# MayDomine/Burst-Attention

Hardware: NVIDIA H100
Metric: attention fwd+bwd TFLOPS/s (bs=1, H=32, d=128, bf16; seq in config, default 262144 on N > 1 GPUs, 65536 on one), aggregate over GPUs (higher is better)
Workload: dtype bf16

## Files before the change

burst-attention_b200/csrc/fwd_sm90.cuh:

```cuda
#pragma once
#include <math.h>
#include <stdlib.h>

#include "host_common.h"
#include "sm90_ptx.cuh"

namespace ba {

constexpr int kBlockM = 128;
constexpr int kBlockN = 128;
constexpr int kKStages = 2;
constexpr int kVStages = 2;
constexpr int kBoxBytes = 128 * 64 * 2;
constexpr int kFwdThreads = 384;

struct FwdParams {
  float* o_acc;
  int64_t oacc_sb, oacc_ss, oacc_sh;
  float* lse;
  int64_t lse_sb, lse_sh;
  void* o_out;
  int64_t oout_sb, oout_ss, oout_sh;
  int B, Sq, Sk, H;
  int G;
  float scale_log2;
  const float* bias;
  int64_t bias_sb, bias_sh;
  int causal;
  int causal_off;
  int load_state;
  int store_lowp;
  int lo;
};

struct __align__(8) FwdBarriers {
  uint64_t q_full;
  uint64_t k_full[kKStages], k_empty[kKStages];
  uint64_t b_full[kKStages];
  uint64_t v_full[kVStages], v_empty[kVStages];
};

template <int kD>
struct FwdLayout {
  static_assert(kD == 64 || kD == 128, "head dim 64 or 128");
  static constexpr uint32_t kTileB = 128 * kD * 2;
  static constexpr int kBoxes = kD / 64;
  static constexpr uint32_t kOffQ = 0;
  static constexpr uint32_t kOffK = kTileB;
  static constexpr uint32_t kOffV = kOffK + kKStages * kTileB;
  static constexpr uint32_t kOffBias = kOffV + kVStages * kTileB;
  static constexpr uint32_t kOffBars = kOffBias + kKStages * kBlockN * 4;
  static constexpr int kSmemBytes = kOffBars + 256 ;
  static_assert(kSmemBytes <= 232448, "forward kernel exceeds 227 KiB of shared memory");
};

__device__ __forceinline__ int fwd_trip_count(int r0, const FwdParams& p) {
  if (r0 >= p.Sq) return 0;
  int r_last = min(r0 + 63, p.Sq - 1);
  int max_limit = p.causal ? min(r_last + p.causal_off, p.Sk - 1) : p.Sk - 1;
  return max_limit < 0 ? 0 : max_limit / kBlockN + 1;
}

__device__ __forceinline__ int fwd_first_tile(int r0, const FwdParams& p) { return max(0, r0 + p.lo) / kBlockN; }

template <bool kBF16, int kD, bool kBias, bool kBand>
__global__ void __launch_bounds__(kFwdThreads, 1)
fwd_chunk_kernel(const __grid_constant__ CUtensorMap tmQ, const __grid_constant__ CUtensorMap tmK,
                 const __grid_constant__ CUtensorMap tmV, const FwdParams p) {
  extern __shared__ __align__(1024) uint8_t smem_raw[];
  uint8_t* smem = smem_raw;
  if ((smem_u32(smem) & 1023u) != 0) __trap();
  using L = FwdLayout<kD>;
  constexpr uint32_t kTileBytes = L::kTileB;
  constexpr int kBoxes = L::kBoxes, kOReg = kD / 2;
  uint8_t* sQ = smem + L::kOffQ;
  uint8_t* sK = smem + L::kOffK;
  uint8_t* sV = smem + L::kOffV;
  float* sBias = reinterpret_cast<float*>(smem + L::kOffBias);
  FwdBarriers* bars = reinterpret_cast<FwdBarriers*>(smem + L::kOffBars);

  const int warp = __shfl_sync(0xffffffffu, threadIdx.x >> 5, 0);
  const int lane = threadIdx.x & 31;
  const int h = blockIdx.y, b = blockIdx.z;
  const int row0 = (p.causal ? (int)(gridDim.x - 1 - blockIdx.x) : (int)blockIdx.x) * kBlockM;
  int n_tiles = max(fwd_trip_count(row0, p), fwd_trip_count(row0 + 64, p));
  int t0 = 0;
  if constexpr (kBand) {
    t0 = min(fwd_first_tile(row0, p), n_tiles);
    n_tiles -= t0;
  }

  if (threadIdx.x == 0) {
    tma_prefetch_desc(&tmQ);
    tma_prefetch_desc(&tmK);
    tma_prefetch_desc(&tmV);
    mbar_init(&bars->q_full, 1);
    for (int i = 0; i < kKStages; ++i) {
      mbar_init(&bars->k_full[i], 1);
      mbar_init(&bars->k_empty[i], 8);
      mbar_init(&bars->b_full[i], 1);
    }
    for (int i = 0; i < kVStages; ++i) {
      mbar_init(&bars->v_full[i], 1);
      mbar_init(&bars->v_empty[i], 8);
    }
    fence_mbar_init();
  }
  __syncthreads();

  if (warp < 4) {
    reg_alloc_dec<40>();
    if (warp != 0) return;
    const int hk = h / p.G;
    if (lane == 0) {
      mbar_arrive_expect_tx(&bars->q_full, kTileBytes);
      for (int half = 0; half < kBoxes; ++half)
        tma_load_4d(sQ + half * kBoxBytes, &tmQ, &bars->q_full, half * 64, h, row0, b);
    }
    for (int i = 0; i < n_tiles; ++i) {
      const int ks = i % kKStages, kph = (i / kKStages) & 1;
      mbar_wait(&bars->k_empty[ks], kph ^ 1);
      if (lane == 0) {
        mbar_arrive_expect_tx(&bars->k_full[ks], kTileBytes);
        for (int half = 0; half < kBoxes; ++half)
          tma_load_4d(sK + ks * kTileBytes + half * kBoxBytes, &tmK, &bars->k_full[ks], half * 64, hk,
                      (t0 + i) * kBlockN, b);
      }
      if constexpr (kBias) {
#pragma unroll
        for (int j = 0; j < 4; ++j) {
          const int key = (t0 + i) * kBlockN + lane + 32 * j;
          float x = 0.f;
          if (key < p.Sk) x = __ldg(p.bias + (int64_t)b * p.bias_sb + (int64_t)h * p.bias_sh + key) * kLog2e;
          sBias[ks * kBlockN + lane + 32 * j] = x;
        }
        __syncwarp();
        if (lane == 0) mbar_arrive(&bars->b_full[ks]);
      }
      if (lane == 0) {
        const int vs = i % kVStages, vph = (i / kVStages) & 1;
        mbar_wait(&bars->v_empty[vs], vph ^ 1);
        mbar_arrive_expect_tx(&bars->v_full[vs], kTileBytes);
        for (int half = 0; half < kBoxes; ++half)
          tma_load_4d(sV + vs * kTileBytes + half * kBoxBytes, &tmV, &bars->v_full[vs], half * 64, hk,
                      (t0 + i) * kBlockN, b);
      }
      __syncwarp();
    }
    return;
  }

  reg_alloc_inc<232>();
  const int wg = (threadIdx.x >> 7) - 1;
  const int w = warp & 3, g = lane >> 2, t = lane & 3;
  const int r_lo = row0 + wg * 64 + 16 * w + g;
  const int rows[2] = {r_lo, r_lo + 8};
  const int n_mine = fwd_trip_count(row0 + wg * 64, p);
  const float scale_log2 = p.scale_log2;
  int limit[2];
#pragma unroll
  for (int r = 0; r < 2; ++r) limit[r] = p.causal ? min(rows[r] + p.causal_off, p.Sk - 1) : p.Sk - 1;
  const int limit_min = min(limit[0], limit[1]);
  int my0 = 0, lo_limit[2] = {0, 0};
  if constexpr (kBand) {
    my0 = fwd_first_tile(row0 + wg * 64, p);
    lo_limit[0] = rows[0] + p.lo;
    lo_limit[1] = rows[1] + p.lo;
  }
  const int lo_limit_max = max(lo_limit[0], lo_limit[1]);

  float o[kOReg];
  float m[2] = {-INFINITY, -INFINITY}, l[2] = {0.f, 0.f};
#pragma unroll
  for (int i = 0; i < kOReg; ++i) o[i] = 0.f;
  if (p.load_state) {
#pragma unroll
    for (int r = 0; r < 2; ++r) {
      if (rows[r] >= p.Sq) continue;
      const float lse_prev = p.lse[(int64_t)b * p.lse_sb + (int64_t)h * p.lse_sh + rows[r]];
      if (lse_prev != -INFINITY) {
        m[r] = lse_prev * kLog2e;
        l[r] = t == 0 ? 1.f : 0.f;
      }
      const float* src = p.o_acc + (int64_t)b * p.oacc_sb + (int64_t)rows[r] * p.oacc_ss + (int64_t)h * p.oacc_sh;
#pragma unroll
      for (int c = 0; c < kD / 8; ++c) {
        const float2 f = __ldg(reinterpret_cast<const float2*>(src + 8 * c + 2 * t));
        o[4 * c + 2 * r] = f.x;
        o[4 * c + 2 * r + 1] = f.y;
      }
    }
  }

  const uint32_t q_base = smem_u32(sQ) + wg * 64 * 128;
  mbar_wait(&bars->q_full, 0);
  for (int i = 0; i < n_tiles; ++i) {
    const int ks = i % kKStages, kph = (i / kKStages) & 1;
    const int vs = i % kVStages, vph = (i / kVStages) & 1;
    const bool work = kBand ? (t0 + i >= my0 && t0 + i < n_mine) : i < n_mine;
    mbar_wait(&bars->k_full[ks], kph);
    float sc[64];
    if (work) {
      const uint32_t k_base = smem_u32(sK + ks * kTileBytes);
      wgmma_fence();
#pragma unroll
      for (int kk = 0; kk < kD / 16; ++kk) {
        const uint32_t off = (kk >> 2) * kBoxBytes + (kk & 3) * 32;
        wgmma_ss_n128<kBF16, 0, 0>(sc, make_desc(q_base + off, 16, 1024), make_desc(k_base + off, 16, 1024),
                                   kk > 0 ? 1u : 0u);
      }
      wgmma_commit();
      wgmma_wait<0>();
      fence_regs<64>(sc);
      const int key0 = (t0 + i) * kBlockN;
      if constexpr (kBias) {
        mbar_wait(&bars->b_full[ks], kph);
        const float* bias = sBias + ks * kBlockN;
#pragma unroll
        for (int c = 0; c < 16; ++c) {
          const float2 bb = *reinterpret_cast<const float2*>(bias + 8 * c + 2 * t);
#pragma unroll
          for (int r = 0; r < 2; ++r) {
            sc[4 * c + 2 * r] = fmaf(sc[4 * c + 2 * r], scale_log2, bb.x);
            sc[4 * c + 2 * r + 1] = fmaf(sc[4 * c + 2 * r + 1], scale_log2, bb.y);
          }
        }
      } else {
#pragma unroll
        for (int j = 0; j < 64; ++j) sc[j] *= scale_log2;
      }
      if (key0 + kBlockN - 1 > limit_min) {
#pragma unroll
        for (int c = 0; c < 16; ++c)
#pragma unroll
          for (int e = 0; e < 4; ++e)
            if (key0 + 8 * c + 2 * t + (e & 1) > limit[e >> 1]) sc[4 * c + e] = -INFINITY;
      }
      if constexpr (kBand) {
        if (key0 < lo_limit_max) {
#pragma unroll
          for (int c = 0; c < 16; ++c)
#pragma unroll
            for (int e = 0; e < 4; ++e)
              if (key0 + 8 * c + 2 * t + (e & 1) < lo_limit[e >> 1]) sc[4 * c + e] = -INFINITY;
        }
      }
    }
    __syncwarp();
    if (lane == 0) mbar_arrive(&bars->k_empty[ks]);
    if (work) {
      uint32_t pa[32];
#pragma unroll
      for (int r = 0; r < 2; ++r) {
        float mx = -INFINITY;
#pragma unroll
        for (int c = 0; c < 16; ++c) mx = fmaxf(mx, fmaxf(sc[4 * c + 2 * r], sc[4 * c + 2 * r + 1]));
        mx = fmaxf(mx, __shfl_xor_sync(0xffffffffu, mx, 1));
        mx = fmaxf(mx, __shfl_xor_sync(0xffffffffu, mx, 2));
        const float m_new = fmaxf(m[r], mx);
        const float f = (m[r] == -INFINITY) ? 0.f : ex2(m[r] - m_new);
        const float neg_m = (m_new == -INFINITY) ? 0.f : -m_new;
        m[r] = m_new;
        float sum = 0.f;
#pragma unroll
        for (int c = 0; c < 16; ++c) {
          const float p0 = ex2(sc[4 * c + 2 * r] + neg_m), p1 = ex2(sc[4 * c + 2 * r + 1] + neg_m);
          sc[4 * c + 2 * r] = p0;
          sc[4 * c + 2 * r + 1] = p1;
          sum += p0 + p1;
        }
        l[r] = l[r] * f + sum;
#pragma unroll
        for (int c = 0; c < kD / 8; ++c) {
          o[4 * c + 2 * r] *= f;
          o[4 * c + 2 * r + 1] *= f;
        }
      }
#pragma unroll
      for (int j = 0; j < 32; ++j) pa[j] = pack2<kBF16>(sc[2 * j], sc[2 * j + 1]);
      mbar_wait(&bars->v_full[vs], vph);
      const uint32_t v_base = smem_u32(sV + vs * kTileBytes);
      fence_regs<32>(pa);
      fence_regs<kOReg>(o);
      wgmma_fence();
#pragma unroll
      for (int kk = 0; kk < kBlockN / 16; ++kk) {
        const uint64_t dv = make_desc(v_base + kk * 16 * 128, kBoxBytes, 1024);
        if constexpr (kD == 128) wgmma_rs_n128<kBF16, 1>(o, pa + 4 * kk, dv, 1u);
        else wgmma_rs_n64<kBF16, 1>(o, pa + 4 * kk, dv, 1u);
      }
      wgmma_commit();
      wgmma_wait<0>();
      fence_regs<kOReg>(o);
    } else {
      mbar_wait(&bars->v_full[vs], vph);
    }
    __syncwarp();
    if (lane == 0) mbar_arrive(&bars->v_empty[vs]);
  }

#pragma unroll
  for (int r = 0; r < 2; ++r) {
    float lr = l[r];
    lr += __shfl_xor_sync(0xffffffffu, lr, 1);
    lr += __shfl_xor_sync(0xffffffffu, lr, 2);
    const int row = rows[r];
    if (row >= p.Sq) continue;
    const float inv_l = lr > 0.f ? 1.f / lr : 0.f;
    if (t == 0) p.lse[(int64_t)b * p.lse_sb + (int64_t)h * p.lse_sh + row] = lr > 0.f ? (m[r] + lg2(lr)) * kLn2 : -INFINITY;
    if (p.store_lowp) {
      uint16_t* dst = reinterpret_cast<uint16_t*>(p.o_out) + (int64_t)b * p.oout_sb + (int64_t)row * p.oout_ss +
                      (int64_t)h * p.oout_sh + 2 * t;
#pragma unroll
      for (int c = 0; c < kD / 8; ++c)
        *reinterpret_cast<uint32_t*>(dst + 8 * c) = pack2<kBF16>(o[4 * c + 2 * r] * inv_l, o[4 * c + 2 * r + 1] * inv_l);
    } else {
      float* dst = p.o_acc + (int64_t)b * p.oacc_sb + (int64_t)row * p.oacc_ss + (int64_t)h * p.oacc_sh + 2 * t;
#pragma unroll
      for (int c = 0; c < kD / 8; ++c)
        *reinterpret_cast<float2*>(dst + 8 * c) = make_float2(o[4 * c + 2 * r] * inv_l, o[4 * c + 2 * r + 1] * inv_l);
    }
  }
}

template <bool kBand>
inline int launch_fwd(int dtype, int D, bool bias, const CUtensorMap& tmQ, const CUtensorMap& tmK,
                      const CUtensorMap& tmV, const FwdParams& p, cudaStream_t stream) {
  const bool bf16 = dtype == BA_DTYPE_BF16;
  void (*kern)(CUtensorMap, CUtensorMap, CUtensorMap, FwdParams);
  if (bias)
    kern = D == 64 ? (bf16 ? fwd_chunk_kernel<true, 64, true, kBand> : fwd_chunk_kernel<false, 64, true, kBand>)
                   : (bf16 ? fwd_chunk_kernel<true, 128, true, kBand> : fwd_chunk_kernel<false, 128, true, kBand>);
  else
    kern = D == 64 ? (bf16 ? fwd_chunk_kernel<true, 64, false, kBand> : fwd_chunk_kernel<false, 64, false, kBand>)
                   : (bf16 ? fwd_chunk_kernel<true, 128, false, kBand> : fwd_chunk_kernel<false, 128, false, kBand>);
  const int smem = D == 64 ? FwdLayout<64>::kSmemBytes : FwdLayout<128>::kSmemBytes;
  BA_CHECK_CUDA(cudaFuncSetAttribute(kern, cudaFuncAttributeMaxDynamicSharedMemorySize, smem));
  dim3 grid((p.Sq + kBlockM - 1) / kBlockM, p.H, p.B);
  kern<<<grid, kFwdThreads, smem, stream>>>(tmQ, tmK, tmV, p);
  BA_CHECK_CUDA(cudaGetLastError());
  return BA_OK;
}

int launch_fwd_band(int dtype, int D, bool bias, const CUtensorMap& tmQ, const CUtensorMap& tmK,
                    const CUtensorMap& tmV, const FwdParams& p, cudaStream_t stream);

}
```

burst-attention_b200/csrc/sm90_ptx.cuh:

```cuda
#pragma once
#include <cuda.h>
#include <cuda_bf16.h>
#include <cuda_fp16.h>
#include <cuda_runtime.h>
#include <stdint.h>

namespace ba {

#define BA_DEVICE __device__ __forceinline__

BA_DEVICE uint32_t smem_u32(const void* p) {
  return static_cast<uint32_t>(__cvta_generic_to_shared(p));
}
constexpr float kLog2e = 1.4426950408889634f;
constexpr float kLn2 = 0.6931471805599453f;
BA_DEVICE float ex2(float x) {
  float y;
  asm("ex2.approx.ftz.f32 %0, %1;" : "=f"(y) : "f"(x));
  return y;
}
BA_DEVICE float lg2(float x) {
  float y;
  asm("lg2.approx.ftz.f32 %0, %1;" : "=f"(y) : "f"(x));
  return y;
}
template <int N>
BA_DEVICE void reg_alloc_inc() {
  asm volatile("setmaxnreg.inc.sync.aligned.u32 %0;" ::"n"(N));
}
template <int N>
BA_DEVICE void reg_alloc_dec() {
  asm volatile("setmaxnreg.dec.sync.aligned.u32 %0;" ::"n"(N));
}

BA_DEVICE void mbar_init(uint64_t* bar, uint32_t count) {
  asm volatile("mbarrier.init.shared::cta.b64 [%0], %1;" ::"r"(smem_u32(bar)), "r"(count));
}
BA_DEVICE void fence_mbar_init() { asm volatile("fence.mbarrier_init.release.cluster;" ::: "memory"); }
BA_DEVICE void mbar_arrive(uint64_t* bar) {
  asm volatile("mbarrier.arrive.shared::cta.b64 _, [%0];" ::"r"(smem_u32(bar)) : "memory");
}
BA_DEVICE void mbar_arrive_expect_tx(uint64_t* bar, uint32_t bytes) {
  asm volatile("mbarrier.arrive.expect_tx.shared::cta.b64 _, [%0], %1;" ::"r"(smem_u32(bar)), "r"(bytes)
               : "memory");
}
BA_DEVICE bool mbar_try_wait(uint64_t* bar, uint32_t parity) {
  uint32_t ok;
  asm volatile(
      "{\n\t.reg .pred p;\n\t"
      "mbarrier.try_wait.parity.shared::cta.b64 p, [%1], %2;\n\t"
      "selp.u32 %0, 1, 0, p;\n\t}\n"
      : "=r"(ok)
      : "r"(smem_u32(bar)), "r"(parity)
      : "memory");
  return ok != 0;
}
BA_DEVICE uint64_t global_ns() {
  uint64_t t;
  asm volatile("mov.u64 %0, %%globaltimer;" : "=l"(t));
  return t;
}
BA_DEVICE void mbar_wait(uint64_t* bar, uint32_t parity) {
  if (mbar_try_wait(bar, parity)) return;
#ifdef BA_NO_WATCHDOG
  while (!mbar_try_wait(bar, parity)) {
  }
#else
  const uint64_t t0 = global_ns();
#pragma unroll 1
  for (;;) {
#pragma unroll 1
    for (int i = 0; i < 1024; ++i)
      if (mbar_try_wait(bar, parity)) return;
    if (global_ns() - t0 > 30000000000ull) break;
  }
  __trap();
#endif
}

BA_DEVICE void fence_proxy_async_smem() { asm volatile("fence.proxy.async.shared::cta;" ::: "memory"); }
BA_DEVICE void named_bar_sync(uint32_t id, uint32_t nthreads) {
  asm volatile("bar.sync %0, %1;" ::"r"(id), "r"(nthreads) : "memory");
}

BA_DEVICE void tma_prefetch_desc(const CUtensorMap* m) {
  asm volatile("prefetch.tensormap [%0];" ::"l"(reinterpret_cast<uint64_t>(m)) : "memory");
}
BA_DEVICE void tma_load_4d(void* smem_dst, const CUtensorMap* m, uint64_t* bar, int c0, int c1, int c2,
                           int c3) {
  asm volatile(
      "cp.async.bulk.tensor.4d.shared::cluster.global.mbarrier::complete_tx::bytes"
      " [%0], [%1, {%3, %4, %5, %6}], [%2];"
      :
      : "r"(smem_u32(smem_dst)), "l"(reinterpret_cast<uint64_t>(m)), "r"(smem_u32(bar)), "r"(c0), "r"(c1),
        "r"(c2), "r"(c3)
      : "memory");
}
BA_DEVICE void tma_reduce_add_4d(const CUtensorMap* m, const void* smem_src, int c0, int c1, int c2, int c3) {
  asm volatile(
      "cp.reduce.async.bulk.tensor.4d.global.shared::cta.add.tile.bulk_group [%0, {%2, %3, %4, %5}], [%1];"
      :
      : "l"(reinterpret_cast<uint64_t>(m)), "r"(smem_u32(smem_src)), "r"(c0), "r"(c1), "r"(c2), "r"(c3)
      : "memory");
}
BA_DEVICE void tma_store_commit() { asm volatile("cp.async.bulk.commit_group;" ::: "memory"); }
template <int N>
BA_DEVICE void tma_store_wait_read() {
  asm volatile("cp.async.bulk.wait_group.read %0;" ::"n"(N) : "memory");
}
template <int N>
BA_DEVICE void tma_store_wait() {
  asm volatile("cp.async.bulk.wait_group %0;" ::"n"(N) : "memory");
}

BA_DEVICE uint64_t make_desc(uint32_t smem_addr, uint32_t lbo_bytes, uint32_t sbo_bytes) {
  uint64_t d = 0;
  d |= static_cast<uint64_t>((smem_addr & 0x3FFFF) >> 4);
  d |= static_cast<uint64_t>((lbo_bytes >> 4) & 0x3FFF) << 16;
  d |= static_cast<uint64_t>((sbo_bytes >> 4) & 0x3FFF) << 32;
  d |= static_cast<uint64_t>(1) << 62;
  return d;
}

BA_DEVICE void wgmma_fence() { asm volatile("wgmma.fence.sync.aligned;" ::: "memory"); }
BA_DEVICE void wgmma_commit() { asm volatile("wgmma.commit_group.sync.aligned;" ::: "memory"); }
template <int N>
BA_DEVICE void wgmma_wait() {
  asm volatile("wgmma.wait_group.sync.aligned %0;" ::"n"(N) : "memory");
}
template <int N>
BA_DEVICE void fence_regs(float* r) {
#pragma unroll
  for (int i = 0; i < N; ++i) asm volatile("" : "+f"(r[i])::"memory");
}
template <int N>
BA_DEVICE void fence_regs(uint32_t* r) {
#pragma unroll
  for (int i = 0; i < N; ++i) asm volatile("" : "+r"(r[i])::"memory");
}

#define BA_WGMMA_ACC_64(d) "+f"(d[0]), "+f"(d[1]), "+f"(d[2]), "+f"(d[3]), "+f"(d[4]), "+f"(d[5]), "+f"(d[6]), "+f"(d[7]), "+f"(d[8]), "+f"(d[9]), "+f"(d[10]), "+f"(d[11]), "+f"(d[12]), "+f"(d[13]), "+f"(d[14]), "+f"(d[15]), "+f"(d[16]), "+f"(d[17]), "+f"(d[18]), "+f"(d[19]), "+f"(d[20]), "+f"(d[21]), "+f"(d[22]), "+f"(d[23]), "+f"(d[24]), "+f"(d[25]), "+f"(d[26]), "+f"(d[27]), "+f"(d[28]), "+f"(d[29]), "+f"(d[30]), "+f"(d[31])
#define BA_WGMMA_ACC_128(d) BA_WGMMA_ACC_64(d), "+f"(d[32]), "+f"(d[33]), "+f"(d[34]), "+f"(d[35]), "+f"(d[36]), "+f"(d[37]), "+f"(d[38]), "+f"(d[39]), "+f"(d[40]), "+f"(d[41]), "+f"(d[42]), "+f"(d[43]), "+f"(d[44]), "+f"(d[45]), "+f"(d[46]), "+f"(d[47]), "+f"(d[48]), "+f"(d[49]), "+f"(d[50]), "+f"(d[51]), "+f"(d[52]), "+f"(d[53]), "+f"(d[54]), "+f"(d[55]), "+f"(d[56]), "+f"(d[57]), "+f"(d[58]), "+f"(d[59]), "+f"(d[60]), "+f"(d[61]), "+f"(d[62]), "+f"(d[63])
#define BA_WGMMA_REGS_64 "%0,%1,%2,%3,%4,%5,%6,%7,%8,%9,%10,%11,%12,%13,%14,%15,%16,%17,%18,%19,%20,%21,%22,%23,%24,%25,%26,%27,%28,%29,%30,%31"
#define BA_WGMMA_REGS_128 BA_WGMMA_REGS_64 ",%32,%33,%34,%35,%36,%37,%38,%39,%40,%41,%42,%43,%44,%45,%46,%47,%48,%49,%50,%51,%52,%53,%54,%55,%56,%57,%58,%59,%60,%61,%62,%63"
#define BA_WGMMA_SS(N, TY, A, B, SC, TA, TB)                                                     \
  asm volatile("{\n\t.reg .pred p;\n\t"                                                        \
               "setp.ne.b32 p, %" #SC ", 0;\n\t"                                               \
               "wgmma.mma_async.sync.aligned.m64n" #N "k16.f32." TY "." TY " "                 \
               "{" BA_WGMMA_REGS_##N "}, "                                                      \
               "%" #A ", %" #B ", p, 1, 1, %" #TA ", %" #TB ";\n\t}\n"                         \
               : BA_WGMMA_ACC_##N(d)                                                            \
               : "l"(a_desc), "l"(b_desc), "r"(scale_d), "n"(kTA), "n"(kTB))
#define BA_WGMMA_RS(N, TY, A0, A1, A2, A3, B, SC, TB)                                            \
  asm volatile("{\n\t.reg .pred p;\n\t"                                                        \
               "setp.ne.b32 p, %" #SC ", 0;\n\t"                                               \
               "wgmma.mma_async.sync.aligned.m64n" #N "k16.f32." TY "." TY " "                 \
               "{" BA_WGMMA_REGS_##N "}, "                                                      \
               "{%" #A0 ",%" #A1 ",%" #A2 ",%" #A3 "}, %" #B ", p, 1, 1, %" #TB ";\n\t}\n"     \
               : BA_WGMMA_ACC_##N(d)                                                            \
               : "r"(a[0]), "r"(a[1]), "r"(a[2]), "r"(a[3]), "l"(b_desc), "r"(scale_d), "n"(kTB))

template <bool kBF16, int kTA, int kTB>
BA_DEVICE void wgmma_ss_n64(float* d, uint64_t a_desc, uint64_t b_desc, uint32_t scale_d) {
  if constexpr (kBF16) BA_WGMMA_SS(64, "bf16", 32, 33, 34, 35, 36);
  else BA_WGMMA_SS(64, "f16", 32, 33, 34, 35, 36);
}
template <bool kBF16, int kTB>
BA_DEVICE void wgmma_rs_n64(float* d, const uint32_t* a, uint64_t b_desc, uint32_t scale_d) {
  if constexpr (kBF16) BA_WGMMA_RS(64, "bf16", 32, 33, 34, 35, 36, 37, 38);
  else BA_WGMMA_RS(64, "f16", 32, 33, 34, 35, 36, 37, 38);
}
template <bool kBF16, int kTA, int kTB>
BA_DEVICE void wgmma_ss_n128(float* d, uint64_t a_desc, uint64_t b_desc, uint32_t scale_d) {
  if constexpr (kBF16) BA_WGMMA_SS(128, "bf16", 64, 65, 66, 67, 68);
  else BA_WGMMA_SS(128, "f16", 64, 65, 66, 67, 68);
}
template <bool kBF16, int kTB>
BA_DEVICE void wgmma_rs_n128(float* d, const uint32_t* a, uint64_t b_desc, uint32_t scale_d) {
  if constexpr (kBF16) BA_WGMMA_RS(128, "bf16", 64, 65, 66, 67, 68, 69, 70);
  else BA_WGMMA_RS(128, "f16", 64, 65, 66, 67, 68, 69, 70);
}

template <bool kBF16>
BA_DEVICE uint32_t pack2(float lo, float hi) {
  if constexpr (kBF16) {
    __nv_bfloat162 v = __floats2bfloat162_rn(lo, hi);
    return *reinterpret_cast<uint32_t*>(&v);
  } else {
    __half2 v = __floats2half2_rn(lo, hi);
    return *reinterpret_cast<uint32_t*>(&v);
  }
}

}
```

Baseline: 504.1.

## Software-pipeline forward QK^T of next tile with PV of current tile

Restructures the consumer loop in the SM90 forward kernel so the S=QK^T wgmma for tile i+1 is issued before the PV wgmma for tile i. The softmax of tile i+1 then runs while the PV matmul is in flight. Non-working tiles are split into leading and trailing pass loops that only cycle the barriers, instead of branching inside the main loop. The producer now issues the K load for tile i+1 ahead of the V load for tile i to feed this ordering. This adds register pressure (sc and pa live across iterations) and more complex barrier ordering.

```diff
diff --git a/burst-attention_b200/csrc/fwd_sm90.cuh b/burst-attention_b200/csrc/fwd_sm90.cuh
--- a/burst-attention_b200/csrc/fwd_sm90.cuh
+++ b/burst-attention_b200/csrc/fwd_sm90.cuh
@@ -117,7 +117,7 @@
       for (int half = 0; half < kBoxes; ++half)
         tma_load_4d(sQ + half * kBoxBytes, &tmQ, &bars->q_full, half * 64, h, row0, b);
     }
-    for (int i = 0; i < n_tiles; ++i) {
+    auto load_k = [&](int i) {
       const int ks = i % kKStages, kph = (i / kKStages) & 1;
       mbar_wait(&bars->k_empty[ks], kph ^ 1);
       if (lane == 0) {
@@ -137,6 +137,10 @@
         __syncwarp();
         if (lane == 0) mbar_arrive(&bars->b_full[ks]);
       }
+    };
+    if (n_tiles > 0) load_k(0);
+    for (int i = 0; i < n_tiles; ++i) {
+      if (i + 1 < n_tiles) load_k(i + 1);
       if (lane == 0) {
         const int vs = i % kVStages, vph = (i / kVStages) & 1;
         mbar_wait(&bars->v_empty[vs], vph ^ 1);
@@ -192,112 +196,156 @@
     }
   }
 
-  const uint32_t q_base = smem_u32(sQ) + wg * 64 * 128;
-  mbar_wait(&bars->q_full, 0);
-  for (int i = 0; i < n_tiles; ++i) {
-    const int ks = i % kKStages, kph = (i / kKStages) & 1;
-    const int vs = i % kVStages, vph = (i / kVStages) & 1;
-    const bool work = kBand ? (t0 + i >= my0 && t0 + i < n_mine) : i < n_mine;
-    mbar_wait(&bars->k_full[ks], kph);
-    float sc[64];
-    if (work) {
-      const uint32_t k_base = smem_u32(sK + ks * kTileBytes);
-      wgmma_fence();
-#pragma unroll
-      for (int kk = 0; kk < kD / 16; ++kk) {
-        const uint32_t off = (kk >> 2) * kBoxBytes + (kk & 3) * 32;
-        wgmma_ss_n128<kBF16, 0, 0>(sc, make_desc(q_base + off, 16, 1024), make_desc(k_base + off, 16, 1024),
-                                   kk > 0 ? 1u : 0u);
-      }
-      wgmma_commit();
-      wgmma_wait<0>();
-      fence_regs<64>(sc);
-      const int key0 = (t0 + i) * kBlockN;
-      if constexpr (kBias) {
-        mbar_wait(&bars->b_full[ks], kph);
-        const float* bias = sBias + ks * kBlockN;
-#pragma unroll
-        for (int c = 0; c < 16; ++c) {
-          const float2 bb = *reinterpret_cast<const float2*>(bias + 8 * c + 2 * t);
-#pragma unroll
-          for (int r = 0; r < 2; ++r) {
-            sc[4 * c + 2 * r] = fmaf(sc[4 * c + 2 * r], scale_log2, bb.x);
-            sc[4 * c + 2 * r + 1] = fmaf(sc[4 * c + 2 * r + 1], scale_log2, bb.y);
-          }
-        }
-      } else {
-#pragma unroll
-        for (int j = 0; j < 64; ++j) sc[j] *= scale_log2;
-      }
-      if (key0 + kBlockN - 1 > limit_min) {
-#pragma unroll
-        for (int c = 0; c < 16; ++c)
-#pragma unroll
-          for (int e = 0; e < 4; ++e)
-            if (key0 + 8 * c + 2 * t + (e & 1) > limit[e >> 1]) sc[4 * c + e] = -INFINITY;
-      }
-      if constexpr (kBand) {
-        if (key0 < lo_limit_max) {
-#pragma unroll
-          for (int c = 0; c < 16; ++c)
-#pragma unroll
-            for (int e = 0; e < 4; ++e)
-              if (key0 + 8 * c + 2 * t + (e & 1) < lo_limit[e >> 1]) sc[4 * c + e] = -INFINITY;
-        }
-      }
-    }
+  int i_begin = 0, i_end = n_mine;
+  if constexpr (kBand) {
+    i_begin = min(my0 - t0, n_tiles);
+    i_end = max(i_begin, n_mine - t0);
+  }
+  auto pass = [&](int i) {
+    const int ks = i % kKStages, vs = i % kVStages;
+    mbar_wait(&bars->k_full[ks], (i / kKStages) & 1);
     __syncwarp();
     if (lane == 0) mbar_arrive(&bars->k_empty[ks]);
-    if (work) {
-      uint32_t pa[32];
-#pragma unroll
-      for (int r = 0; r < 2; ++r) {
-        float mx = -INFINITY;
-#pragma unroll
-        for (int c = 0; c < 16; ++c) mx = fmaxf(mx, fmaxf(sc[4 * c + 2 * r], sc[4 * c + 2 * r + 1]));
-        mx = fmaxf(mx, __shfl_xor_sync(0xffffffffu, mx, 1));
-        mx = fmaxf(mx, __shfl_xor_sync(0xffffffffu, mx, 2));
-        const float m_new = fmaxf(m[r], mx);
-        const float f = (m[r] == -INFINITY) ? 0.f : ex2(m[r] - m_new);
-        const float neg_m = (m_new == -INFINITY) ? 0.f : -m_new;
-        m[r] = m_new;
-        float sum = 0.f;
-#pragma unroll
-        for (int c = 0; c < 16; ++c) {
-          const float p0 = ex2(sc[4 * c + 2 * r] + neg_m), p1 = ex2(sc[4 * c + 2 * r + 1] + neg_m);
-          sc[4 * c + 2 * r] = p0;
-          sc[4 * c + 2 * r + 1] = p1;
-          sum += p0 + p1;
+    mbar_wait(&bars->v_full[vs], (i / kVStages) & 1);
+    __syncwarp();
+    if (lane == 0) mbar_arrive(&bars->v_empty[vs]);
+  };
+
+  const uint32_t q_base = smem_u32(sQ) + wg * 64 * 128;
+  float sc[64];
+  uint32_t pa[32];
+  float f[2];
+  auto issue_s = [&](int i) {
+    const int ks = i % kKStages;
+    mbar_wait(&bars->k_full[ks], (i / kKStages) & 1);
+    const uint32_t k_base = smem_u32(sK + ks * kTileBytes);
+    wgmma_fence();
+#pragma unroll
+    for (int kk = 0; kk < kD / 16; ++kk) {
+      const uint32_t off = (kk >> 2) * kBoxBytes + (kk & 3) * 32;
+      wgmma_ss_n128<kBF16, 0, 0>(sc, make_desc(q_base + off, 16, 1024), make_desc(k_base + off, 16, 1024),
+                                 kk > 0 ? 1u : 0u);
+    }
+    wgmma_commit();
+  };
+  auto wait_v = [&](int i) { mbar_wait(&bars->v_full[i % kVStages], (i / kVStages) & 1); };
+  auto issue_pv = [&](int i) {
+    const int vs = i % kVStages;
+    const uint32_t v_base = smem_u32(sV + vs * kTileBytes);
+    fence_regs<32>(pa);
+    fence_regs<kOReg>(o);
+    wgmma_fence();
+#pragma unroll
+    for (int kk = 0; kk < kBlockN / 16; ++kk) {
+      const uint64_t dv = make_desc(v_base + kk * 16 * 128, kBoxBytes, 1024);
+      if constexpr (kD == 128) wgmma_rs_n128<kBF16, 1>(o, pa + 4 * kk, dv, 1u);
+      else wgmma_rs_n64<kBF16, 1>(o, pa + 4 * kk, dv, 1u);
+    }
+    wgmma_commit();
+  };
+  auto softmax = [&](int i) {
+    const int ks = i % kKStages;
+    const int key0 = (t0 + i) * kBlockN;
+    if constexpr (kBias) {
+      mbar_wait(&bars->b_full[ks], (i / kKStages) & 1);
+      const float* bias = sBias + ks * kBlockN;
+#pragma unroll
+      for (int c = 0; c < 16; ++c) {
+        const float2 bb = *reinterpret_cast<const float2*>(bias + 8 * c + 2 * t);
+#pragma unroll
+        for (int r = 0; r < 2; ++r) {
+          sc[4 * c + 2 * r] = fmaf(sc[4 * c + 2 * r], scale_log2, bb.x);
+          sc[4 * c + 2 * r + 1] = fmaf(sc[4 * c + 2 * r + 1], scale_log2, bb.y);
         }
-        l[r] = l[r] * f + sum;
-#pragma unroll
-        for (int c = 0; c < kD / 8; ++c) {
-          o[4 * c + 2 * r] *= f;
-          o[4 * c + 2 * r + 1] *= f;
-        }
-      }
-#pragma unroll
-      for (int j = 0; j < 32; ++j) pa[j] = pack2<kBF16>(sc[2 * j], sc[2 * j + 1]);
-      mbar_wait(&bars->v_full[vs], vph);
-      const uint32_t v_base = smem_u32(sV + vs * kTileBytes);
-      fence_regs<32>(pa);
-      fence_regs<kOReg>(o);
-      wgmma_fence();
-#pragma unroll
-      for (int kk = 0; kk < kBlockN / 16; ++kk) {
-        const uint64_t dv = make_desc(v_base + kk * 16 * 128, kBoxBytes, 1024);
-        if constexpr (kD == 128) wgmma_rs_n128<kBF16, 1>(o, pa + 4 * kk, dv, 1u);
-        else wgmma_rs_n64<kBF16, 1>(o, pa + 4 * kk, dv, 1u);
-      }
-      wgmma_commit();
+      }
+    } else {
+#pragma unroll
+      for (int j = 0; j < 64; ++j) sc[j] *= scale_log2;
+    }
+    if (key0 + kBlockN - 1 > limit_min) {
+#pragma unroll
+      for (int c = 0; c < 16; ++c)
+#pragma unroll
+        for (int e = 0; e < 4; ++e)
+          if (key0 + 8 * c + 2 * t + (e & 1) > limit[e >> 1]) sc[4 * c + e] = -INFINITY;
+    }
+    if constexpr (kBand) {
+      if (key0 < lo_limit_max) {
+#pragma unroll
+        for (int c = 0; c < 16; ++c)
+#pragma unroll
+          for (int e = 0; e < 4; ++e)
+            if (key0 + 8 * c + 2 * t + (e & 1) < lo_limit[e >> 1]) sc[4 * c + e] = -INFINITY;
+      }
+    }
+    __syncwarp();
+    if (lane == 0) mbar_arrive(&bars->k_empty[ks]);
+#pragma unroll
+    for (int r = 0; r < 2; ++r) {
+      float mx = -INFINITY;
+#pragma unroll
+      for (int c = 0; c < 16; ++c) mx = fmaxf(mx, fmaxf(sc[4 * c + 2 * r], sc[4 * c + 2 * r + 1]));
+      mx = fmaxf(mx, __shfl_xor_sync(0xffffffffu, mx, 1));
+      mx = fmaxf(mx, __shfl_xor_sync(0xffffffffu, mx, 2));
+      const float m_new = fmaxf(m[r], mx);
+      f[r] = (m[r] == -INFINITY) ? 0.f : ex2(m[r] - m_new);
+      const float neg_m = (m_new == -INFINITY) ? 0.f : -m_new;
+      m[r] = m_new;
+      float sum = 0.f;
+#pragma unroll
+      for (int c = 0; c < 16; ++c) {
+        const float p0 = ex2(sc[4 * c + 2 * r] + neg_m), p1 = ex2(sc[4 * c + 2 * r + 1] + neg_m);
+        sc[4 * c + 2 * r] = p0;
+        sc[4 * c + 2 * r + 1] = p1;
+        sum += p0 + p1;
+      }
+      l[r] = l[r] * f[r] + sum;
+    }
+  };
+  auto rescale_pack = [&]() {
+#pragma unroll
+    for (int r = 0; r < 2; ++r)
+#pragma unroll
+      for (int c = 0; c < kD / 8; ++c) {
+        o[4 * c + 2 * r] *= f[r];
+        o[4 * c + 2 * r + 1] *= f[r];
+      }
+#pragma unroll
+    for (int j = 0; j < 32; ++j) pa[j] = pack2<kBF16>(sc[2 * j], sc[2 * j + 1]);
+  };
+  auto release_v = [&](int i) {
+    __syncwarp();
+    if (lane == 0) mbar_arrive(&bars->v_empty[i % kVStages]);
+  };
+
+  mbar_wait(&bars->q_full, 0);
+  for (int i = 0; i < i_begin; ++i) pass(i);
+  if (i_begin < i_end) {
+    issue_s(i_begin);
+    wgmma_wait<0>();
+    fence_regs<64>(sc);
+    softmax(i_begin);
+    wait_v(i_begin);
+    rescale_pack();
+    for (int i = i_begin; i + 1 < i_end; ++i) {
+      issue_s(i + 1);
+      issue_pv(i);
+      wgmma_wait<1>();
+      fence_regs<64>(sc);
+      softmax(i + 1);
+      wait_v(i + 1);
       wgmma_wait<0>();
       fence_regs<kOReg>(o);
-    } else {
-      mbar_wait(&bars->v_full[vs], vph);
-    }
-    __syncwarp();
-    if (lane == 0) mbar_arrive(&bars->v_empty[vs]);
-  }
+      fence_regs<32>(pa);
+      release_v(i);
+      rescale_pack();
+    }
+    issue_pv(i_end - 1);
+    wgmma_wait<0>();
+    fence_regs<kOReg>(o);
+    release_v(i_end - 1);
+  }
+  for (int i = i_end; i < n_tiles; ++i) pass(i);
 
 #pragma unroll
   for (int r = 0; r < 2; ++r) {
```

Result: no change. 507.8, median of 6 (+0.7%).

## Share K/V tile loads across 2-CTA clusters via TMA multicast in forward kernel

Applied to the files above, without the earlier changes.

Launches the forward kernel with 2-CTA clusters so neighbouring query tiles share K/V loads. CTA rank 0 multicasts K and rank 1 multicasts V to both CTAs, and consumers release stage buffers in both CTAs through cluster-scoped mbarrier arrivals. Each pair iterates over the longer of the two CTAs' KV ranges, and cluster syncs are added at setup and teardown. The aim is to halve L2 to SMEM traffic for K/V. The cost is lockstep coupling between paired CTAs, extra work on causal pairs, and cross-CTA synchronisation overhead.

```diff
diff --git a/burst-attention_b200/csrc/fwd_sm90.cuh b/burst-attention_b200/csrc/fwd_sm90.cuh
--- a/burst-attention_b200/csrc/fwd_sm90.cuh
+++ b/burst-attention_b200/csrc/fwd_sm90.cuh
@@ -82,11 +82,16 @@
   const int warp = __shfl_sync(0xffffffffu, threadIdx.x >> 5, 0);
   const int lane = threadIdx.x & 31;
   const int h = blockIdx.y, b = blockIdx.z;
-  const int row0 = (p.causal ? (int)(gridDim.x - 1 - blockIdx.x) : (int)blockIdx.x) * kBlockM;
-  int n_tiles = max(fwd_trip_count(row0, p), fwd_trip_count(row0 + 64, p));
+  const uint32_t rank = cluster_ctarank();
+  const int q_tile = p.causal ? (int)(gridDim.x - 1 - blockIdx.x) : (int)blockIdx.x;
+  const int row0 = q_tile * kBlockM;
+  const int pair_row0 = (q_tile & ~1) * kBlockM;
+  int n_tiles = 0;
+#pragma unroll
+  for (int r = 0; r < 4; ++r) n_tiles = max(n_tiles, fwd_trip_count(pair_row0 + 64 * r, p));
   int t0 = 0;
   if constexpr (kBand) {
-    t0 = min(fwd_first_tile(row0, p), n_tiles);
+    t0 = min(fwd_first_tile(pair_row0, p), n_tiles);
     n_tiles -= t0;
   }
 
@@ -97,56 +102,60 @@
     mbar_init(&bars->q_full, 1);
     for (int i = 0; i < kKStages; ++i) {
       mbar_init(&bars->k_full[i], 1);
-      mbar_init(&bars->k_empty[i], 8);
+      mbar_init(&bars->k_empty[i], 16);
       mbar_init(&bars->b_full[i], 1);
     }
     for (int i = 0; i < kVStages; ++i) {
       mbar_init(&bars->v_full[i], 1);
-      mbar_init(&bars->v_empty[i], 8);
+      mbar_init(&bars->v_empty[i], 16);
     }
     fence_mbar_init();
   }
-  __syncthreads();
+  cluster_sync();
 
   if (warp < 4) {
     reg_alloc_dec<40>();
-    if (warp != 0) return;
-    const int hk = h / p.G;
-    if (lane == 0) {
-      mbar_arrive_expect_tx(&bars->q_full, kTileBytes);
-      for (int half = 0; half < kBoxes; ++half)
-        tma_load_4d(sQ + half * kBoxBytes, &tmQ, &bars->q_full, half * 64, h, row0, b);
-    }
-    for (int i = 0; i < n_tiles; ++i) {
-      const int ks = i % kKStages, kph = (i / kKStages) & 1;
-      mbar_wait(&bars->k_empty[ks], kph ^ 1);
+    if (warp == 0) {
+      const int hk = h / p.G;
       if (lane == 0) {
-        mbar_arrive_expect_tx(&bars->k_full[ks], kTileBytes);
+        mbar_arrive_expect_tx(&bars->q_full, kTileBytes);
         for (int half = 0; half < kBoxes; ++half)
-          tma_load_4d(sK + ks * kTileBytes + half * kBoxBytes, &tmK, &bars->k_full[ks], half * 64, hk,
-                      (t0 + i) * kBlockN, b);
-      }
-      if constexpr (kBias) {
-#pragma unroll
-        for (int j = 0; j < 4; ++j) {
-          const int key = (t0 + i) * kBlockN + lane + 32 * j;
-          float x = 0.f;
-          if (key < p.Sk) x = __ldg(p.bias + (int64_t)b * p.bias_sb + (int64_t)h * p.bias_sh + key) * kLog2e;
-          sBias[ks * kBlockN + lane + 32 * j] = x;
+          tma_load_4d(sQ + half * kBoxBytes, &tmQ, &bars->q_full, half * 64, h, row0, b);
+      }
+      for (int i = 0; i < n_tiles; ++i) {
+        const int ks = i % kKStages, kph = (i / kKStages) & 1;
+        mbar_wait(&bars->k_empty[ks], kph ^ 1);
+        if (lane == 0) {
+          mbar_arrive_expect_tx(&bars->k_full[ks], kTileBytes);
+          if (rank == 0)
+            for (int half = 0; half < kBoxes; ++half)
+              tma_load_4d_multicast(sK + ks * kTileBytes + half * kBoxBytes, &tmK, &bars->k_full[ks], 0x3,
+                                    half * 64, hk, (t0 + i) * kBlockN, b);
+        }
+        if constexpr (kBias) {
+#pragma unroll
+          for (int j = 0; j < 4; ++j) {
+            const int key = (t0 + i) * kBlockN + lane + 32 * j;
+            float x = 0.f;
+            if (key < p.Sk) x = __ldg(p.bias + (int64_t)b * p.bias_sb + (int64_t)h * p.bias_sh + key) * kLog2e;
+            sBias[ks * kBlockN + lane + 32 * j] = x;
+          }
+          __syncwarp();
+          if (lane == 0) mbar_arrive(&bars->b_full[ks]);
+        }
+        if (lane == 0) {
+          const int vs = i % kVStages, vph = (i / kVStages) & 1;
+          mbar_wait(&bars->v_empty[vs], vph ^ 1);
+          mbar_arrive_expect_tx(&bars->v_full[vs], kTileBytes);
+          if (rank == 1)
+            for (int half = 0; half < kBoxes; ++half)
+              tma_load_4d_multicast(sV + vs * kTileBytes + half * kBoxBytes, &tmV, &bars->v_full[vs], 0x3,
+                                    half * 64, hk, (t0 + i) * kBlockN, b);
         }
         __syncwarp();
-        if (lane == 0) mbar_arrive(&bars->b_full[ks]);
-      }
-      if (lane == 0) {
-        const int vs = i % kVStages, vph = (i / kVStages) & 1;
-        mbar_wait(&bars->v_empty[vs], vph ^ 1);
-        mbar_arrive_expect_tx(&bars->v_full[vs], kTileBytes);
-        for (int half = 0; half < kBoxes; ++half)
-          tma_load_4d(sV + vs * kTileBytes + half * kBoxBytes, &tmV, &bars->v_full[vs], half * 64, hk,
-                      (t0 + i) * kBlockN, b);
-      }
-      __syncwarp();
-    }
+      }
+    }
+    cluster_sync();
     return;
   }
 
@@ -247,7 +256,10 @@
       }
     }
     __syncwarp();
-    if (lane == 0) mbar_arrive(&bars->k_empty[ks]);
+    if (lane == 0) {
+      mbar_arrive_cluster(&bars->k_empty[ks], 0);
+      mbar_arrive_cluster(&bars->k_empty[ks], 1);
+    }
     if (work) {
       uint32_t pa[32];
 #pragma unroll
@@ -296,7 +308,10 @@
       mbar_wait(&bars->v_full[vs], vph);
     }
     __syncwarp();
-    if (lane == 0) mbar_arrive(&bars->v_empty[vs]);
+    if (lane == 0) {
+      mbar_arrive_cluster(&bars->v_empty[vs], 0);
+      mbar_arrive_cluster(&bars->v_empty[vs], 1);
+    }
   }
 
 #pragma unroll
@@ -321,6 +336,7 @@
         *reinterpret_cast<float2*>(dst + 8 * c) = make_float2(o[4 * c + 2 * r] * inv_l, o[4 * c + 2 * r + 1] * inv_l);
     }
   }
+  cluster_sync();
 }
 
 template <bool kBand>
@@ -336,8 +352,17 @@
                    : (bf16 ? fwd_chunk_kernel<true, 128, false, kBand> : fwd_chunk_kernel<false, 128, false, kBand>);
   const int smem = D == 64 ? FwdLayout<64>::kSmemBytes : FwdLayout<128>::kSmemBytes;
   BA_CHECK_CUDA(cudaFuncSetAttribute(kern, cudaFuncAttributeMaxDynamicSharedMemorySize, smem));
-  dim3 grid((p.Sq + kBlockM - 1) / kBlockM, p.H, p.B);
-  kern<<<grid, kFwdThreads, smem, stream>>>(tmQ, tmK, tmV, p);
+  cudaLaunchConfig_t cfg = {};
+  cfg.gridDim = dim3(((p.Sq + kBlockM - 1) / kBlockM + 1) & ~1, p.H, p.B);
+  cfg.blockDim = dim3(kFwdThreads);
+  cfg.dynamicSmemBytes = smem;
+  cfg.stream = stream;
+  cudaLaunchAttribute cluster;
+  cluster.id = cudaLaunchAttributeClusterDimension;
+  cluster.val.clusterDim.x = 2, cluster.val.clusterDim.y = 1, cluster.val.clusterDim.z = 1;
+  cfg.attrs = &cluster;
+  cfg.numAttrs = 1;
+  BA_CHECK_CUDA(cudaLaunchKernelEx(&cfg, kern, tmQ, tmK, tmV, p));
   BA_CHECK_CUDA(cudaGetLastError());
   return BA_OK;
 }
diff --git a/burst-attention_b200/csrc/sm90_ptx.cuh b/burst-attention_b200/csrc/sm90_ptx.cuh
--- a/burst-attention_b200/csrc/sm90_ptx.cuh
+++ b/burst-attention_b200/csrc/sm90_ptx.cuh
@@ -78,6 +78,23 @@
 #endif
 }
 
+BA_DEVICE uint32_t cluster_ctarank() {
+  uint32_t r;
+  asm volatile("mov.u32 %0, %%cluster_ctarank;" : "=r"(r));
+  return r;
+}
+BA_DEVICE void cluster_sync() {
+  asm volatile("barrier.cluster.arrive.release;\n\tbarrier.cluster.wait.acquire;" ::: "memory");
+}
+BA_DEVICE void mbar_arrive_cluster(uint64_t* bar, uint32_t cta) {
+  asm volatile(
+      "{\n\t.reg .b32 remote;\n\t"
+      "mapa.shared::cluster.u32 remote, %0, %1;\n\t"
+      "mbarrier.arrive.shared::cluster.b64 _, [remote];\n\t}\n" ::"r"(smem_u32(bar)),
+      "r"(cta)
+      : "memory");
+}
+
 BA_DEVICE void fence_proxy_async_smem() { asm volatile("fence.proxy.async.shared::cta;" ::: "memory"); }
 BA_DEVICE void named_bar_sync(uint32_t id, uint32_t nthreads) {
   asm volatile("bar.sync %0, %1;" ::"r"(id), "r"(nthreads) : "memory");
@@ -94,6 +111,16 @@
       :
       : "r"(smem_u32(smem_dst)), "l"(reinterpret_cast<uint64_t>(m)), "r"(smem_u32(bar)), "r"(c0), "r"(c1),
         "r"(c2), "r"(c3)
+      : "memory");
+}
+BA_DEVICE void tma_load_4d_multicast(void* smem_dst, const CUtensorMap* m, uint64_t* bar, uint16_t cta_mask, int c0,
+                                     int c1, int c2, int c3) {
+  asm volatile(
+      "cp.async.bulk.tensor.4d.shared::cluster.global.mbarrier::complete_tx::bytes.multicast::cluster"
+      " [%0], [%1, {%4, %5, %6, %7}], [%2], %3;"
+      :
+      : "r"(smem_u32(smem_dst)), "l"(reinterpret_cast<uint64_t>(m)), "r"(smem_u32(bar)), "h"(cta_mask), "r"(c0),
+        "r"(c1), "r"(c2), "r"(c3)
       : "memory");
 }
 BA_DEVICE void tma_reduce_add_4d(const CUtensorMap* m, const void* smem_src, int c0, int c1, int c2, int c3) {
```

Measured after the change: 509.8 before, 513.8 after, median of 6. About the same (+0.8%).
